# CNR-STIIMA-IRAS/rosdyn

Hardware: AMD Instinct MI355X
Metric: RNEA+regressor evals/s (6-DOF, batch 1e6) (higher is better)
Workload: dtype f64; 1 GPU; configs[1]: 6-DOF chain (ur10_like base_link->wrist_3_link, n=6, P=60), batch 1000000 samples per GPU, fp64 getJointTorque + dense getRegressor, inputs sample-major, Y layout stacked; samples_per_gpu=1000000, n_active=6, n_params=60, parallelism=sample-sharded x1

## Files before the change

### rosdyn_amd/csrc/rdyn_cholqr.hip

```cpp
#include <hip/hip_runtime.h>
#include <cstdint>
#include <type_traits>
#include "rdyn_device.h"
#include "rdyn_devmath.h"
#include "rdyn_kernels.h"
#include "rdyn_gram_common.h"
#include "rdyn_duo_common.h"
#include "rdyn_launch_util.h"

#ifndef RDYN_CHOLQR_AHEAD
#define RDYN_CHOLQR_AHEAD 2
#endif
#define DUO_BARRIER_LDS() asm volatile("s_waitcnt lgkmcnt(0)\n\ts_barrier" ::: "memory")
#define DUO_BARRIER() asm volatile("s_barrier" ::: "memory")

namespace
{

typedef const __attribute__((address_space(1))) double* GlobalD;

template <int NJ, bool ALLREV, int NPAIR, bool WGLOBAL, int XB, int KIN = 0>
__global__ __launch_bounds__(128 * NPAIR) void k_regressor_pgram(const RdynLdsGramArgs fa, const double* __restrict__ Wg, const int* __restrict__ run_flag)
{
  constexpr bool DIRECT = true;
  constexpr int NB = (10 * NJ + 1 + 15) / 16 + XB, NT = NB * (NB + 1) / 2, P = 10 * NJ;
  constexpr int SH = XB > 0 ? 0 : 16 * NB - (P + 1);
  constexpr int WB = WGLOBAL ? 0 : NT * 2048;
  if (run_flag && *run_flag == 0) return;
  extern __shared__ __attribute__((aligned(32))) char lds_raw[];
  const int lane = threadIdx.x & 63;
  const int wave = __builtin_amdgcn_readfirstlane(threadIdx.x >> 6);
  const bool sweeper = wave < NPAIR;
  const int pair = NPAIR == 4 ? (wave & 3) : NPAIR == 2 ? (wave & 1) : (wave < 3 ? wave : (wave == 3 ? 2 : wave - 4));
  if constexpr (!WGLOBAL)
  {
    double* const wl = (double*)lds_raw;
    for (int i = threadIdx.x; i < NT * 256; i += 128 * NPAIR) wl[i] = Wg[i];
    __syncthreads();
  }
  char* const tile = lds_raw + WB + (size_t)pair * fa.tile_bytes;
  const int n = fa.n_active;
  const int64_t t_mul = fa.tile_stride > 1 ? fa.tile_stride : 1;
  const int64_t n_tiles = ((fa.n_samples + 15) / 16 + t_mul - 1) / t_mul;
  const int64_t t_step = (int64_t)gridDim.x * NPAIR;
  const int64_t t_first = (int64_t)blockIdx.x * NPAIR + pair;
  const int64_t trips_raw = (n_tiles - (int64_t)blockIdx.x * NPAIR + t_step - 1) / t_step;
  const int64_t trips = trips_raw > 0 ? trips_raw : 0;

#ifndef RDYN_PGRAM_X_IDLE
#define RDYN_PGRAM_X_IDLE(wave_) true
#endif
#ifdef RDYN_PGRAM_X_NOSWEEP
  if (sweeper && RDYN_PGRAM_X_IDLE(wave))
  {
    if (KIN) DUO_BARRIER();
    for (int64_t it = 0; it < trips; ++it)
      for (int f = 0; f <= NJ; ++f) DUO_BARRIER_LDS();
  }
  else
#endif
  if (sweeper && KIN)
  {
    constexpr int XV = NJ <= 6 ? 21 : 12;
    constexpr int KIN_SLOTS = 3;
    const int KIN_SW = wave;
    char* const kin_tiles = lds_raw + WB;
    double* const kin_xch_base = (double*)(lds_raw + WB + (size_t)4 * fa.tile_bytes);
#include "rdyn_kin_sweepers.inc"
  }
  else if (sweeper)
  {
    ChainPtr c = as_const(fa.chain);
    const int s_loc = lane >> 2, k = lane & 3;
    const int r0 = k, r1 = k + 4;
    RDYN_DUO_INPUT_OFFSETS(fa, k, in_oa, in_ob);
    const int fB = 4;
    double nqa = 0.0, ndqa = 0.0, nddqa = 0.0, nqb = 0.0, ndqb = 0.0, nddqb = 0.0, nb0 = 0.0, nb1 = 0.0;
    auto fetch = [&](int64_t tile_index) {
      int64_t sx = tile_index * t_mul * 16 + s_loc;
      if (sx >= fa.n_samples) sx = fa.n_samples - 1;
      const int64_t o = sx * fa.in_ss;
      if (fa.bcol)
      {
        if (r0 < n) nb0 = fa.bcol[o + in_oa];
        if (r1 < n) nb1 = fa.bcol[o + in_ob];
      }
      if (k < n)
      {
        nqa = fa.q[o + in_oa];
        ndqa = fa.dq[o + in_oa];
        nddqa = fa.ddq[o + in_oa];
      }
      if (k + 4 < n)
      {
        nqb = fa.q[o + in_ob];
        ndqb = fa.dq[o + in_ob];
        nddqb = fa.ddq[o + in_ob];
      }
    };
    if (t_first < n_tiles) fetch(t_first);
    for (int64_t it = 0; it < trips; ++it)
    {
      const int64_t tl = t_first + it * t_step;
      const bool valid = tl < n_tiles && tl * t_mul * 16 + s_loc < fa.n_samples;
      const int m0idx = valid ? r0 : -2, m1idx = valid ? r1 : -2;
      const double qa = nqa, dqa = ndqa, ddqa = nddqa, qb = nqb, dqb = ndqb, ddqb = nddqb;
      const double tb0 = valid ? nb0 : 0.0, tb1 = valid ? nb1 : 0.0;
      if (tl + t_step < n_tiles) fetch(tl + t_step);
      double sna, csa, snb, csb;
      rdyn_sincos(qa, &sna, &csa);
      rdyn_sincos(qb, &snb, &csb);
      const double oca = 1.0 - csa, ocb = 1.0 - csb;
      V3 w = mk(0, 0, 0), vl = mk(0, 0, 0), al = mk(0, 0, 0);
      V3 lin = mk(-c->g[0], -c->g[1], -c->g[2]);
      V3 L0 = mk(0, 0, 0), A0 = mk(0, 0, 0), L1 = mk(0, 0, 0), A1 = mk(0, 0, 0);
#pragma unroll
      for (int f = 0; f < NJ; ++f)
      {
#include "rdyn_duo_link_body.inc"
      }
      if constexpr (XB > 0)
      {
#include "rdyn_duo_comp_cols.inc"
      }
      {
        char* const lb = tile + fa.lds_off_b + s_loc * 8;
        if (r0 < n) *(double*)(lb + r0 * 128) = tb0;
        if (r1 < n) *(double*)(lb + r1 * 128) = tb1;
      }
      DUO_BARRIER_LDS();
    }
  }
  else
  {
#ifdef RDYN_CHOLQR_MFMA_PRIO
    __builtin_amdgcn_s_setprio(RDYN_CHOLQR_MFMA_PRIO);
#endif
    const int cl = lane & 15, g = lane >> 4;
    constexpr int X0 = (P + SH) / 4, NX = 4 * NB - X0;
    const int K = XB > 0 ? fa.n_comp_cols : 0;
    int xoff[NX], xrow[NX];
#pragma unroll
    for (int i = 0; i < NX; ++i)
    {
      const int col = 4 * (X0 + i) + g - SH;
      int off = 0, row = -2;
      if (col >= P && col < P + K)
      {
        row = fa.comp_col_row[col - P];
        off = fa.lds_off_c + (col - P) * fa.comp_stride - row * 128;
      }
      else if (col == P + K)
      {
        off = fa.lds_off_b;
        row = -1;
      }
      xoff[i] = off + cl * 8;
      xrow[i] = row;
    }
    auto a_operand = [&](int cb1, int kk, int j) -> double {
      const int id = 4 * cb1 + kk, col = 4 * id + g - SH;
      double a = 0.0;
      if (id < X0 || (4 * id - SH < P && col < P))
      {
        if (col < 0) return 0.0;
        const int f = (col * 205) >> 11;
        constexpr int PAD = KIN ? KIN : 4;
        const int off = f * (640 * f + 640 + 80 * PAD) + (col - 10 * f) * (128 * f + 128 + 8 * PAD);
        if (j <= f) a = *(const double*)(tile + off + cl * 8 + j * 128);
      }
      else
      {
        const int i = id - X0;
        if (xrow[i] == -1 || xrow[i] == j) a = *(const double*)(tile + xoff[i] + j * 128);
      }
      return a;
    };
    d4 acc[NT];
#pragma unroll
    for (int t = 0; t < NT; ++t) acc[t] = (d4){0.0, 0.0, 0.0, 0.0};
    const char* const wl = lds_raw + lane * 8;
    GlobalD wgp = (GlobalD)Wg;
#ifdef RDYN_PGRAM_X_NOW
    auto wglob = [&](int blk_kk) -> double { return (double)(blk_kk + lane); };
#else
    auto wglob = [&](int blk_kk) -> double { return (wgp + blk_kk * 64)[lane]; };
#endif
    d4 D[NB];
    auto stage1 = [&](int j, int band) {
#pragma unroll
      for (int cb = 0; cb < NB; ++cb) D[cb] = (d4){0.0, 0.0, 0.0, 0.0};
      constexpr int AH = RDYN_CHOLQR_AHEAD;
      double ring[AH + 1][NB], aring[AH + 1];
      if constexpr (WGLOBAL) asm volatile("" : "+s"(wgp));
      auto load_row = [&](int r, double (&dst)[NB], double& adst) {
        const int c1 = band + (r >> 2), k4 = r & 3;
        adst = c1 < NB ? a_operand(c1, k4, j) : 0.0;
#pragma unroll
        for (int cb2 = 0; cb2 < NB; ++cb2)
        {
          dst[cb2] = 0.0;
          if (c1 < NB && cb2 >= c1)
          {
            if constexpr (WGLOBAL) dst[cb2] = wglob((cb2 * (cb2 + 1) / 2 + c1) * 4 + k4);
            else dst[cb2] = *(const double*)(wl + ((cb2 * (cb2 + 1) / 2 + c1) * 4 + k4) * 512);
          }
        }
      };
#pragma unroll
      for (int r = 0; r < AH; ++r) load_row(r, ring[r], aring[r]);
#pragma unroll
      for (int cb1 = 0; cb1 < NB; ++cb1)
      {
        if (cb1 < band) continue;
#pragma unroll
        for (int kk = 0; kk < 4; ++kk)
        {
          const int r = (cb1 - band) * 4 + kk;
          load_row(r + AH, ring[(r + AH) % (AH + 1)], aring[(r + AH) % (AH + 1)]);
          asm volatile("" ::: "memory");
          const double a = aring[r % (AH + 1)];
#pragma unroll
          for (int cb2 = cb1; cb2 < NB; ++cb2) D[cb2] = __builtin_amdgcn_mfma_f64_16x16x4f64(a, ring[r % (AH + 1)][cb2], D[cb2], 0, 0, 0);
        }
      }
    };
    auto stage2 = [&](int band) {
#pragma unroll
      for (int t = 0; t < 4; ++t)
      {
        int ti = 0;
#pragma unroll
        for (int cb = 0; cb < NB; ++cb)
#pragma unroll
          for (int rb = 0; rb <= cb; ++rb)
          {
            if (rb >= band) acc[ti] = __builtin_amdgcn_mfma_f64_16x16x4f64(D[rb][t], D[cb][t], acc[ti], 0, 0, 0);
            ++ti;
          }
      }
    };
    if (KIN) DUO_BARRIER();
    for (int64_t it = 0; it <= trips; ++it)
    {
#ifdef RDYN_PGRAM_X_NOMFMA
      const bool have = it > trips + 1;
#else
      const bool have = it > 0;
#endif
#pragma unroll
      for (int f = 0; f < NJ; ++f)
      {
        if (have) stage1(f, (SH + 10 * f) >> 4);
        if (it < trips) DUO_BARRIER_LDS();
        else asm volatile("s_waitcnt lgkmcnt(0)" ::: "memory");
        if (have) stage2((SH + 10 * f) >> 4);
      }
      if (it < trips) DUO_BARRIER_LDS();
    }
    DUO_BARRIER_LDS();
    double* red = (double*)lds_raw;
    for (int w = 0; w < NPAIR; ++w)
    {
      if (pair == w)
      {
#pragma unroll
        for (int t = 0; t < NT; ++t)
#pragma unroll
          for (int r = 0; r < 4; ++r)
          {
            const int idx = t * 256 + ((g + 4 * r) * 16 + cl);
            red[idx] = (w == 0) ? acc[t][r] : red[idx] + acc[t][r];
          }
      }
      asm volatile("s_waitcnt lgkmcnt(0)" ::: "memory");
      __builtin_amdgcn_s_barrier();
    }
  }
  if (sweeper)
    for (int w = 0; w < NPAIR + 1; ++w) __builtin_amdgcn_s_barrier();
  asm volatile("" ::: "memory");
  {
    const double* red = (const double*)lds_raw;
    double* slab = fa.slabs + (int64_t)blockIdx.x * (NT * 256);
    for (int i = threadIdx.x; i < NT * 256; i += 128 * NPAIR) slab[i] = red[i];
  }
}

template <int NB>
__global__ __launch_bounds__(256) void k_pgram_rows(const double* __restrict__ A, const double* __restrict__ bvec, int64_t rows, int64_t lda, int n_cols,
                                                    const double* __restrict__ Wg, double* __restrict__ slabs, const int* __restrict__ run_flag)
{
  constexpr int NT = NB * (NB + 1) / 2;
  if (run_flag && *run_flag == 0) return;
  extern __shared__ __attribute__((aligned(32))) char lds_raw[];
  const int lane = threadIdx.x & 63;
  const int wave = __builtin_amdgcn_readfirstlane(threadIdx.x >> 6);
  const int cl = lane & 15, g = lane >> 4;
  {
    double* const wl = (double*)lds_raw;
    for (int i = threadIdx.x; i < NT * 256; i += 256) wl[i] = Wg[i];
    __syncthreads();
  }
  d4 acc[NT];
#pragma unroll
  for (int t = 0; t < NT; ++t) acc[t] = (d4){0.0, 0.0, 0.0, 0.0};
  const char* const wl = lds_raw + lane * 8;
  const int64_t gstride = (int64_t)gridDim.x * 4 * 16;
  int64_t r0 = ((int64_t)blockIdx.x * 4 + wave) * 16;
  double cur[4 * NB], nxt[4 * NB];
  const double* const base = A + (int64_t)g * lda;
  const int id_b = bvec ? n_cols >> 2 : -1, g_b = n_cols & 3;
  auto load = [&](int64_t rbase, double (&v)[4 * NB]) {
    const int64_t r = rbase + cl;
    const bool in = r < rows;
    const double* pcol = base + r;
#pragma unroll
    for (int id = 0; id < 4 * NB; ++id)
    {
      double x = 0.0;
      if (in && 4 * id + g < n_cols) x = *pcol;
      if (id == id_b && in && g == g_b) x = bvec[r];
      v[id] = x;
      pcol += 4 * lda;
      asm volatile("" : "+v"(pcol));
    }
  };
  if (r0 < rows) load(r0, cur);
  while (r0 < rows)
  {
    const int64_t rn = r0 + gstride;
    constexpr bool LATE = NB >= 7;
    if (!LATE && rn < rows) load(rn, nxt);
    d4 D[NB];
#pragma unroll
    for (int cb = 0; cb < NB; ++cb) D[cb] = (d4){0.0, 0.0, 0.0, 0.0};
    {
      constexpr int AH = LATE ? 1 : 2;
      double ring[AH + 1][NB];
      auto load_row = [&](int r, double (&dst)[NB]) {
        const int c1 = r >> 2, k4 = r & 3;
#pragma unroll
        for (int cb2 = 0; cb2 < NB; ++cb2)
        {
          dst[cb2] = 0.0;
          if (c1 < NB && cb2 >= c1) dst[cb2] = *(const double*)(wl + ((cb2 * (cb2 + 1) / 2 + c1) * 4 + k4) * 512);
        }
      };
#pragma unroll
      for (int r = 0; r < AH; ++r) load_row(r, ring[r]);
#pragma unroll
      for (int cb1 = 0; cb1 < NB; ++cb1)
#pragma unroll
        for (int kk = 0; kk < 4; ++kk)
        {
          const int r = cb1 * 4 + kk;
          load_row(r + AH, ring[(r + AH) % (AH + 1)]);
          asm volatile("" ::: "memory");
          const double a = cur[r];
#pragma unroll
          for (int cb2 = cb1; cb2 < NB; ++cb2) D[cb2] = __builtin_amdgcn_mfma_f64_16x16x4f64(a, ring[r % (AH + 1)][cb2], D[cb2], 0, 0, 0);
        }
    }
    if (LATE)
    {
      asm volatile("" ::: "memory");
      if (rn < rows) load(rn, nxt);
// ... 1049 lines not shown
```

### rosdyn_amd/csrc/rdyn_duo_gram.hip

```cpp
#include <hip/hip_runtime.h>
#include <cstdint>
#include "rdyn_device.h"
#include "rdyn_devmath.h"
#include "rdyn_kernels.h"
#include "rdyn_gram_common.h"
#include "rdyn_duo_common.h"
#include "rdyn_launch_util.h"

#ifndef RDYN_DUO_SWEEP_UNROLL
#define RDYN_DUO_SWEEP_UNROLL 1
#endif

namespace
{

#ifdef RDYN_DUO_STAMPS
#ifndef RDYN_DUO_STAMP_TRIP
#define RDYN_DUO_STAMP_TRIP 7
#endif
#define DUO_STAMP_DECL unsigned long long st_wait = 0, st_t0 = __builtin_amdgcn_s_memtime(), st_tmp; long long st_it = -1; int st_n = 0
#define DUO_STAMP_TRIP(it_) st_it = (it_)
#define DUO_STAMP_MARK(t_) do { if (blockIdx.x == 0 && st_it == RDYN_DUO_STAMP_TRIP && (threadIdx.x & 63) == 0 && st_n < 32) fa.slabs[(int64_t)600 * 4096 + (threadIdx.x >> 6) * 32 + st_n++] = (double)((t_) - st_t0); } while (0)
#define DUO_STAMP_HERE(wait_lds) do { if (wait_lds) asm volatile("s_waitcnt lgkmcnt(0)" ::: "memory"); DUO_STAMP_MARK(__builtin_amdgcn_s_memtime()); } while (0)
#define DUO_BARRIER_LDS() do { st_tmp = __builtin_amdgcn_s_memtime(); DUO_STAMP_MARK(st_tmp); asm volatile("s_waitcnt lgkmcnt(0)\n\ts_barrier" ::: "memory"); const unsigned long long st_e = __builtin_amdgcn_s_memtime(); st_wait += st_e - st_tmp; DUO_STAMP_MARK(st_e); } while (0)
#define DUO_BARRIER() do { st_tmp = __builtin_amdgcn_s_memtime(); DUO_STAMP_MARK(st_tmp); asm volatile("s_barrier" ::: "memory"); const unsigned long long st_e = __builtin_amdgcn_s_memtime(); st_wait += st_e - st_tmp; DUO_STAMP_MARK(st_e); } while (0)
#define DUO_STAMP_OUT(NT_) do { if (lane == 0) { double* o = fa.slabs + ((int64_t)(256 + blockIdx.x) * (NT_ * 256)) + wave * 2; o[0] = (double)(__builtin_amdgcn_s_memtime() - st_t0); o[1] = (double)st_wait; } } while (0)
#else
#define DUO_STAMP_DECL
#define DUO_STAMP_TRIP(it_)
#define DUO_STAMP_HERE(wait_lds)
#define DUO_BARRIER_LDS() asm volatile("s_waitcnt lgkmcnt(0)\n\ts_barrier" ::: "memory")
#define DUO_BARRIER() asm volatile("s_barrier" ::: "memory")
#define DUO_STAMP_OUT(NT_)
#endif

typedef double d4h __attribute__((ext_vector_type(4), aligned(16)));

template <int NJ, bool DIRECT, int XB, bool ALLREV, int KIN = 0>
__global__ __launch_bounds__(KIN ? 768 : 512) void k_regressor_gram_duo(const RdynLdsGramArgs fa)
{
  constexpr int NB = (10 * NJ + 1 + 15) / 16 + XB;
  constexpr int NT = NB * (NB + 1) / 2;
  constexpr int P = 10 * NJ;
  extern __shared__ __attribute__((aligned(32))) char lds_raw[];
  const int lane = threadIdx.x & 63;
  const int wave = __builtin_amdgcn_readfirstlane(threadIdx.x >> 6);
  constexpr int NSW = KIN ? 8 : 4;
  const int pair = KIN ? (wave - NSW) & 3 : wave & 3;
  const bool sweeper = wave < NSW;
  char* const tile = lds_raw + (size_t)pair * fa.tile_bytes;
  const int n = fa.n_active;
  const int64_t t_mul = fa.tile_stride > 1 ? fa.tile_stride : 1;
  const int64_t n_tiles = ((fa.n_samples + 15) / 16 + t_mul - 1) / t_mul;
  const int64_t t_step = (int64_t)gridDim.x * 4;
  const int64_t t_first = (int64_t)blockIdx.x * 4 + pair;
  const int64_t trips_raw = (n_tiles - (int64_t)blockIdx.x * 4 + t_step - 1) / t_step;
  const int64_t trips = trips_raw > 0 ? trips_raw : 0;
  DUO_STAMP_DECL;

  if (sweeper && KIN)
  {
    constexpr int XV = NJ <= 6 ? (XB > 0 ? 30 : 21) : 12;
    constexpr int KIN_SLOTS = 2;
    const int KIN_SW = wave;
    char* const kin_tiles = lds_raw;
    double* const kin_xch_base = (double*)(lds_raw + (size_t)4 * fa.tile_bytes);
#include "rdyn_kin_sweepers.inc"
  }
  else if (sweeper)
  {
    ChainPtr c = as_const(fa.chain);
#ifdef RDYN_DUO_SWEEP_PRIO
    __builtin_amdgcn_s_setprio(RDYN_DUO_SWEEP_PRIO);
#endif
    const int s_loc = lane >> 2, k = lane & 3;
    const int r0 = k, r1 = k + 4;
    RDYN_DUO_INPUT_OFFSETS(fa, k, in_oa, in_ob);
    int fB = DIRECT ? 4 : NJ;
    if (!DIRECT)
      for (int f = NJ - 1; f >= 0; --f)
        if (fa.lds_m[f] >= 5) fB = f;
    double nqa = 0.0, ndqa = 0.0, nddqa = 0.0, nqb = 0.0, ndqb = 0.0, nddqb = 0.0, nb0 = 0.0, nb1 = 0.0;
    auto fetch = [&](int64_t tile_index) {
      int64_t sx = tile_index * t_mul * 16 + s_loc;
      if (sx >= fa.n_samples) sx = fa.n_samples - 1;
      const int64_t o = sx * fa.in_ss;
      if (fa.bcol)
      {
        if (r0 < n) nb0 = fa.bcol[o + in_oa];
        if (r1 < n) nb1 = fa.bcol[o + in_ob];
      }
      if (k < n)
      {
        nqa = fa.q[o + in_oa];
        ndqa = fa.dq[o + in_oa];
        nddqa = fa.ddq[o + in_oa];
      }
      if (k + 4 < n)
      {
        nqb = fa.q[o + in_ob];
        ndqb = fa.dq[o + in_ob];
        nddqb = fa.ddq[o + in_ob];
      }
    };
    if (t_first < n_tiles) fetch(t_first);
    for (int64_t it = 0; it < trips; ++it)
    {
      const int64_t tl = t_first + it * t_step;
      const bool valid = tl < n_tiles && tl * t_mul * 16 + s_loc < fa.n_samples;
      const int m0idx = valid ? r0 : -2, m1idx = valid ? r1 : -2;
      const double qa = nqa, dqa = ndqa, ddqa = nddqa, qb = nqb, dqb = ndqb, ddqb = nddqb;
      const double tb0 = valid ? nb0 : 0.0, tb1 = valid ? nb1 : 0.0;
      if (tl + t_step < n_tiles) fetch(tl + t_step);
      double sna, csa, snb, csb;
      rdyn_sincos(qa, &sna, &csa);
      rdyn_sincos(qb, &snb, &csb);
      const double oca = 1.0 - csa, ocb = 1.0 - csb;

      V3 w = mk(0, 0, 0), vl = mk(0, 0, 0), al = mk(0, 0, 0);
      V3 lin = mk(-c->g[0], -c->g[1], -c->g[2]);
      V3 L0 = mk(0, 0, 0), A0 = mk(0, 0, 0), L1 = mk(0, 0, 0), A1 = mk(0, 0, 0);
      if constexpr (DIRECT)
      {
#pragma unroll
        for (int f = 0; f < NJ; ++f)
        {
#include "rdyn_duo_link_body.inc"
        }
      }
      else
      {
#pragma unroll 1
        for (int f = 0; f < NJ; ++f)
        {
#include "rdyn_duo_link_body.inc"
        }
      }
      if (XB > 0 || fa.n_comps > 0)
      {
#include "rdyn_duo_comp_cols.inc"
      }
      {
        char* const lb = tile + fa.lds_off_b + s_loc * 8;
        if (r0 < n) *(double*)(lb + r0 * 128) = tb0;
        if (r1 < n) *(double*)(lb + r1 * 128) = tb1;
      }
      DUO_BARRIER_LDS();
    }
  }
  else
  {
#ifdef RDYN_DUO_MFMA_PRIO
    __builtin_amdgcn_s_setprio(RDYN_DUO_MFMA_PRIO);
#endif
    const int cl = lane & 15, g = lane >> 4;
    int colbase[NB], colm[NB], collo[NB];
    const int K = XB > 0 ? fa.n_comp_cols : 0;
    const int KF = K;
#pragma unroll
    for (int cb = 0; cb < NB; ++cb)
    {
      const int pp = 16 * cb + cl;
      const int pl = pp - KF - 1;
      const int p = pp < KF ? P + pp : (pp == KF ? P + K : (pl >= P ? P + K + 1 : 10 * (NJ - 1 - pl / 10) + pl % 10));
      int base = 0, hi = 0, lo = 0;
      if (p < P)
      {
        const int f = p / 10;
        base = fa.lds_off[f] + (p - 10 * f) * fa.lds_stride[f];
        hi = fa.lds_m[f];
      }
      else if (p < P + K)
      {
        lo = fa.comp_col_row[p - P];
        hi = lo + 1;
        base = fa.lds_off_c + (p - P) * fa.comp_stride - lo * 128;
      }
      else if (p == P + K)
      {
        base = fa.lds_off_b;
        hi = n;
      }
      colbase[cb] = base + g * 32;
      colm[cb] = hi;
      collo[cb] = lo;
    }
    d4 acc[NT];
#pragma unroll
    for (int t = 0; t < NT; ++t) acc[t] = (d4){0.0, 0.0, 0.0, 0.0};
    auto lds_group = [&](int j, int band, d4* op) {
#pragma unroll
      for (int cb = 0; cb < NB; ++cb)
      {
        d4 x = (d4){0.0, 0.0, 0.0, 0.0};
        if (cb <= band && j < colm[cb] && j >= collo[cb]) x = *(const d4h*)(tile + colbase[cb] + j * 128);
        op[cb] = x;
      }
    };
    auto mfma_band = [&](const d4* op, int band) {
#pragma unroll
      for (int t = 0; t < 4; ++t)
      {
        int ti = 0;
#pragma unroll
        for (int cb = 0; cb < NB; ++cb)
#pragma unroll
          for (int rb = 0; rb <= cb; ++rb)
          {
#ifdef RDYN_DUO_4X4_TIMING
            if (cb <= band)
            {
              acc[ti][0] = __builtin_amdgcn_mfma_f64_4x4x4f64(op[rb][t], op[cb][t], acc[ti][0], 0, 0, 0);
              acc[ti][1] = __builtin_amdgcn_mfma_f64_4x4x4f64(op[rb][t], op[cb][t], acc[ti][1], 0, 0, 0);
              acc[ti][2] = __builtin_amdgcn_mfma_f64_4x4x4f64(op[rb][t], op[cb][t], acc[ti][2], 0, 0, 0);
              if (rb != cb) acc[ti][3] = __builtin_amdgcn_mfma_f64_4x4x4f64(op[rb][t], op[cb][t], acc[ti][3], 0, 0, 0);
            }
#else
            if (cb <= band) acc[ti] = __builtin_amdgcn_mfma_f64_16x16x4f64(op[rb][t], op[cb][t], acc[ti], 0, 0, 0);
#endif
            ++ti;
          }
      }
    };
    constexpr bool ONEBUF = (NJ >= 7 && XB > 0) || KIN != 0;
    d4 opa[NB], opb[ONEBUF ? 1 : NB];
    if (KIN) DUO_BARRIER();
    for (int64_t it = 0; it <= trips; ++it)
    {
      DUO_STAMP_TRIP(it);
      const bool have = it > 0;
      if (have) lds_group(0, (KF + 10 * NJ) >> 4, opa);
#pragma unroll
      for (int f = 0; f < NJ; ++f)
      {
        d4* const cur = (ONEBUF || !(f & 1)) ? opa : opb;
        d4* const nxt = (ONEBUF || (f & 1)) ? opa : opb;
        if (it < trips) DUO_BARRIER_LDS();
        else asm volatile("s_waitcnt lgkmcnt(0)" ::: "memory");
        if (have)
        {
          if constexpr (ONEBUF)
          {
            mfma_band(cur, (KF + 10 * (NJ - f)) >> 4);
            if (f + 1 < NJ) lds_group(f + 1, (KF + 10 * (NJ - f - 1)) >> 4, nxt);
          }
          else
          {
            if (f + 1 < NJ) lds_group(f + 1, (KF + 10 * (NJ - f - 1)) >> 4, nxt);
            mfma_band(cur, (KF + 10 * (NJ - f)) >> 4);
          }
        }
      }
      if (it < trips) DUO_BARRIER_LDS();
    }

    DUO_STAMP_OUT(NT);
    DUO_BARRIER_LDS();
    double* red = (double*)lds_raw;
    const int cw = wave - NSW;
    for (int w = 0; w < 4; ++w)
    {
      if (cw == w)
      {
#pragma unroll
        for (int t = 0; t < NT; ++t)
#pragma unroll
          for (int r = 0; r < 4; ++r)
          {
            const int idx = t * 256 + ((g + 4 * r) * 16 + cl);
            red[idx] = (w == 0) ? acc[t][r] : red[idx] + acc[t][r];
          }
      }
      asm volatile("s_waitcnt lgkmcnt(0)" ::: "memory");
      __builtin_amdgcn_s_barrier();
    }
  }
  if (sweeper)
  {
    DUO_STAMP_OUT(NT);
    for (int w = 0; w < 5; ++w) __builtin_amdgcn_s_barrier();
  }
  asm volatile("" ::: "memory");
  {
    const double* red = (const double*)lds_raw;
    double* slab = fa.slabs + (int64_t)blockIdx.x * (NT * 256);
    for (int i = threadIdx.x; i < NT * 256; i += (KIN ? 768 : 512)) slab[i] = red[i];
  }
}

template <int NJ, bool DIRECT, int XB, bool ALLREV = false, int KIN = 0>
hipError_t launch_duo_nj2(const RdynLdsGramArgs& a, int blocks, size_t lds_bytes, hipStream_t st)
{
  hipError_t e = opt_in_lds_once<k_regressor_gram_duo<NJ, DIRECT, XB, ALLREV, KIN>>();
  if (e != hipSuccess) return e;
  hipLaunchKernelGGL((k_regressor_gram_duo<NJ, DIRECT, XB, ALLREV, KIN>), dim3(blocks), dim3(KIN ? 768 : 512), lds_bytes, st, a);
  return hipGetLastError();
}
template <int NJ>
hipError_t launch_duo_nj(const RdynLdsGramArgs& a, int blocks, size_t lds_bytes, hipStream_t st)
{
  bool direct = a.n_active == NJ;
  for (int f = 0; direct && f < NJ; ++f) direct = a.lds_m[f] == f + 1 && a.first_col[f] == 10 * f && a.lds_stride[f] == (16 * (f + 1) + 4) * 8;
  const int xb = a.n_comp_cols > 0 ? 1 : 0;
  if (a.sweep_lanes)
  {
    bool compact = a.n_active == NJ;
    for (int f = 0; compact && f < NJ; ++f) compact = a.lds_m[f] == f + 1 && a.first_col[f] == 10 * f && a.lds_stride[f] == (16 * (f + 1) + 2) * 8;
    if constexpr (NJ <= 6)
    {
      if (direct && xb == 0) return a.all_revolute ? launch_duo_nj2<NJ, true, 0, true, 4>(a, blocks, lds_bytes, st) : launch_duo_nj2<NJ, true, 0, false, 4>(a, blocks, lds_bytes, st);
      if constexpr (NJ >= 5)
        if (direct && xb == 1) return a.all_revolute ? launch_duo_nj2<NJ, true, 1, true, 4>(a, blocks, lds_bytes, st) : launch_duo_nj2<NJ, true, 1, false, 4>(a, blocks, lds_bytes, st);
    }
    else if (compact && xb == 0)
      return a.all_revolute ? launch_duo_nj2<NJ, true, 0, true, 2>(a, blocks, lds_bytes, st) : launch_duo_nj2<NJ, true, 0, false, 2>(a, blocks, lds_bytes, st);
    return hipErrorInvalidValue;
  }
  if (xb == 0 && direct && a.all_revolute) return launch_duo_nj2<NJ, true, 0, true>(a, blocks, lds_bytes, st);
  if (xb == 0) return direct ? launch_duo_nj2<NJ, true, 0>(a, blocks, lds_bytes, st) : launch_duo_nj2<NJ, false, 0>(a, blocks, lds_bytes, st);
  if constexpr (NJ >= 5)
  {
    if (xb == 1 && direct && a.all_revolute) return launch_duo_nj2<NJ, true, 1, true>(a, blocks, lds_bytes, st);
    if (xb == 1) return direct ? launch_duo_nj2<NJ, true, 1>(a, blocks, lds_bytes, st) : launch_duo_nj2<NJ, false, 1>(a, blocks, lds_bytes, st);
  }
  return hipErrorInvalidValue;
}
}

bool rdyn_regressor_gram_duo_supported(int n_cols) { return n_cols >= 20 && n_cols <= 70; }
int rdyn_regressor_gram_duo_kin_pad(int n_joints, int n_comp_cols)
{
  if (n_joints >= 2 && n_joints <= 6) return (n_comp_cols == 0 || n_joints >= 5) ? 4 : 0;
  return (n_joints == 7 && n_comp_cols == 0) ? 2 : 0;
}
bool rdyn_regressor_gram_duo_supports_components(int n_cols, int n_comp_cols)
{
  if (!rdyn_regressor_gram_duo_supported(n_cols) || n_comp_cols < 0 || n_comp_cols > 96) return false;
  if (n_comp_cols == 0) return true;
  const int nb1 = (n_cols + 1 + 15) / 16 + 1;
  return n_cols >= 50 && n_cols + n_comp_cols + 1 <= 16 * nb1;
}

hipError_t rdyn_launch_regressor_gram_duo(int n_cols, const RdynLdsGramArgs& a, int blocks, size_t lds_bytes, hipStream_t st)
{
#define CALL(N) launch_duo_nj<N>(a, blocks, lds_bytes, st)
  RDYN_DISPATCH_JOINTS_2_7(n_cols / 10, CALL)
#undef CALL
}
```

### rosdyn_amd/csrc/rdyn_kin_link_body.inc

```
        asm volatile("" : "+s"(c));
        JointRef J = c->j[g];
        const int type = J.type;
        const bool rev = ALLREV || type == RDYN_REVOLUTE, pri = !ALLREV && type == RDYN_PRISMATIC;
        const double qf = q_[g], dqf = dq_[g], ddqf = ddq_[g];
        {
          const int64_t oj = o_next + (int64_t)fa.in_map[g] * fa.in_sj;
          q_[g] = fa.q[oj];
          dq_[g] = fa.dq[oj];
          ddq_[g] = fa.ddq[oj];
        }
        const double sn = rev ? sn_[g] : 0.0, oc = rev ? oc_[g] : 0.0;
        const double qp = pri ? qf : 0.0;
        double R[9];
#pragma unroll
        for (int i = 0; i < 9; ++i) R[i] = fma(sn, J.B[i], fma(oc, J.C[i], J.A[i]));
        const V3 tt = ALLREV ? ld3(J.t) : axpy(ld3(J.t), ld3(J.up), qp);
        {
          const V3 wn = rotT(R, w);
          const V3 vn = rotT(R, vl + cross(w, tt));
          const V3 aln = rotT(R, al);
          const V3 an = rotT(R, lin + cross(al, tt));
          w = wn; vl = vn; al = aln; lin = an;
        }
        const V3 u = ld3(J.u);
        {
          const double dqr = rev ? dqf : 0.0, ddqr = rev ? ddqf : 0.0, dqp = pri ? dqf : 0.0, ddqp = pri ? ddqf : 0.0;
          const V3 wxu = cross(w, u);
          if constexpr (ALLREV)
            lin = axpy(lin, cross(vl, u), dqr);
          else
            lin = axpy(axpy(axpy(lin, cross(vl, u), dqr), wxu, dqp), u, ddqp);
          al = axpy(axpy(al, wxu, dqr), u, ddqr);
          w = axpy(w, u, dqr);
          if constexpr (!ALLREV) vl = axpy(vl, u, dqp);
        }
        const V3 d = lin + cross(w, vl);
        double* const o = xch + (g & 1) * (XV * 64);
        if constexpr (XV == 12)
        {
          o[0] = sn; o[64] = oc; o[128] = qp;
          o[192] = w.x; o[256] = w.y; o[320] = w.z;
          o[384] = al.x; o[448] = al.y; o[512] = al.z;
          o[576] = d.x; o[640] = d.y; o[704] = d.z;
        }
        else
        {
          const double wxy = w.x * w.y, wxz = w.x * w.z, wyz = w.y * w.z;
          const double wxx = w.x * w.x, wyy = w.y * w.y, wzz = w.z * w.z;
#pragma unroll
          for (int i = 0; i < 9; ++i) o[i * 64] = R[i];
          o[576] = tt.x; o[640] = tt.y; o[704] = tt.z;
          o[768] = w.x; o[832] = w.y; o[896] = w.z;
          o[960] = al.x; o[1024] = al.y; o[1088] = al.z;
          o[1152] = d.x; o[1216] = d.y; o[1280] = d.z;
          if constexpr (XV == 30)
          {
            o[1344] = -(wyy + wzz); o[1408] = wxy - al.z; o[1472] = wxz + al.y;
            o[1536] = wxy + al.z; o[1600] = -(wxx + wzz); o[1664] = wyz - al.x;
            o[1728] = wxz - al.y; o[1792] = wyz + al.x; o[1856] = -(wxx + wyy);
          }
        }
```

### rosdyn_amd/csrc/rdyn_kin_sweepers.inc

```
#ifndef DUO_STAMP_TRIP
#define DUO_STAMP_TRIP(it_)
#endif
#ifndef DUO_STAMP_HERE
#define DUO_STAMP_HERE(wait_lds)
#endif
    ChainPtr c = as_const(fa.chain);
    const int sub = lane >> 4, s_loc = lane & 15;
    char* const tile = kin_tiles + (size_t)sub * fa.tile_bytes;
    double* const xch = kin_xch_base + lane;
    const int64_t t_mine = (int64_t)blockIdx.x * 4 + sub;
    auto sample_offset = [&](int64_t tile_index) -> int64_t {
      if (tile_index >= n_tiles) tile_index = n_tiles - 1;
      int64_t sx = tile_index * t_mul * 16 + s_loc;
      if (sx >= fa.n_samples) sx = fa.n_samples - 1;
      return sx * fa.in_ss;
    };
    if (KIN_SW == 0)
    {
      double q_[NJ], dq_[NJ], ddq_[NJ];
      {
        const int64_t o = sample_offset(t_mine);
#pragma unroll
        for (int j = 0; j < NJ; ++j)
        {
          const int64_t oj = o + (int64_t)fa.in_map[j] * fa.in_sj;
          q_[j] = fa.q[oj];
          dq_[j] = fa.dq[oj];
          ddq_[j] = fa.ddq[oj];
        }
      }
      V3 w = mk(0, 0, 0), vl = mk(0, 0, 0), al = mk(0, 0, 0), lin = mk(-c->g[0], -c->g[1], -c->g[2]);
      int64_t o_next = sample_offset(t_mine + t_step);
      double sn_[NJ], oc_[NJ];
#define RDYN_KIN_ONE_SINCOS(j_)                                                                     \
  do                                                                                               \
  {                                                                                                \
    double sn1_, cs1_;                                                                             \
    rdyn_sincos_small(q_[j_], &sn1_, &cs1_);                                                       \
    if (__builtin_expect(!(fabs(q_[j_]) <= 1048576.0), 0))                                         \
    {                                                                                              \
      const DuoSinCos big_ = duo_sincos_cold(q_[j_]);                                              \
      sn1_ = big_.sn;                                                                              \
      cs1_ = big_.cs;                                                                              \
    }                                                                                              \
    sn_[j_] = sn1_;                                                                                \
    oc_[j_] = 1.0 - cs1_;                                                                          \
  } while (0)
#pragma unroll
      for (int j = 0; j < NJ; ++j) RDYN_KIN_ONE_SINCOS(j);
      {
        constexpr int g = 0;
#include "rdyn_kin_link_body.inc"
      }
      DUO_BARRIER_LDS();
      for (int64_t it = 0; it < trips; ++it)
      {
        DUO_STAMP_TRIP(it);
#pragma unroll
        for (int f = 0; f < NJ; ++f)
        {
          if (f + 1 < NJ)
          {
            const int g = f + 1;
#include "rdyn_kin_link_body.inc"
          }
          else
          {
#pragma unroll
            for (int j = 0; j < NJ; ++j) RDYN_KIN_ONE_SINCOS(j);
          }
          DUO_BARRIER_LDS();
        }
        w = mk(0, 0, 0); vl = mk(0, 0, 0); al = mk(0, 0, 0); lin = mk(-c->g[0], -c->g[1], -c->g[2]);
        o_next = sample_offset(t_mine + (it + 2) * t_step);
        {
          constexpr int g = 0;
#include "rdyn_kin_link_body.inc"
        }
        DUO_BARRIER_LDS();
      }
    }
    else
    {
      constexpr int S = KIN_SLOTS;
      int r[S];
      int64_t ob[S];
#pragma unroll
      for (int k = 0; k < S; ++k)
      {
        r[k] = fa.sw_rows[3 * (KIN_SW - 1) + k];
        ob[k] = r[k] < 8 ? (int64_t)fa.in_map[r[k]] * fa.in_sj : 0;
      }
      double nb[S], nq[S], nd[S];
#pragma unroll
      for (int k = 0; k < S; ++k) nb[k] = nq[k] = nd[k] = 0.0;
      auto fetch = [&](int64_t tile_index) {
        const int64_t o = sample_offset(tile_index);
#pragma unroll
        for (int k = 0; k < S; ++k)
        {
          if (fa.bcol && r[k] < 8) nb[k] = fa.bcol[o + ob[k]];
          if ((XB > 0 || fa.n_comps > 0) && r[k] < 8)
          {
            nq[k] = fa.q[o + ob[k]];
            nd[k] = fa.dq[o + ob[k]];
          }
        }
      };
      fetch(t_mine);
      DUO_BARRIER();
      for (int64_t it = 0; it < trips; ++it)
      {
        DUO_STAMP_TRIP(it);
        const int64_t tl = t_mine + it * t_step;
        const bool valid = tl < n_tiles && tl * t_mul * 16 + s_loc < fa.n_samples;
        double tb[S], qr[S], dqr[S];
#pragma unroll
        for (int k = 0; k < S; ++k)
        {
          tb[k] = valid ? nb[k] : 0.0;
          qr[k] = nq[k];
          dqr[k] = nd[k];
        }
        fetch(tl + t_step);
        V3 L[S], A[S];
#pragma unroll
        for (int k = 0; k < S; ++k) L[k] = A[k] = mk(0, 0, 0);
        int col_off = 0;
#pragma unroll 1
        for (int f = 0; f < NJ; ++f)
        {
          const double* const xi = xch + (f & 1) * (XV * 64);
          double R[9], b00, b01, b02, b10, b11, b12, b20, b21, b22;
          V3 tt, w, al, d;
          if constexpr (XV == 12)
          {
            asm volatile("" : "+s"(c));
            JointRef J = c->j[f];
            const double sn = xi[0], oc = xi[64], qp = xi[128];
            w = mk(xi[192], xi[256], xi[320]);
            al = mk(xi[384], xi[448], xi[512]);
            d = mk(xi[576], xi[640], xi[704]);
#pragma unroll
            for (int i = 0; i < 9; ++i) R[i] = fma(sn, J.B[i], fma(oc, J.C[i], J.A[i]));
            tt = ALLREV ? ld3(J.t) : axpy(ld3(J.t), ld3(J.up), qp);
            const double wxy = w.x * w.y, wxz = w.x * w.z, wyz = w.y * w.z;
            const double wxx = w.x * w.x, wyy = w.y * w.y, wzz = w.z * w.z;
            b00 = -(wyy + wzz); b01 = wxy - al.z; b02 = wxz + al.y;
            b10 = wxy + al.z; b11 = -(wxx + wzz); b12 = wyz - al.x;
            b20 = wxz - al.y; b21 = wyz + al.x; b22 = -(wxx + wyy);
          }
          else
          {
#pragma unroll
            for (int i = 0; i < 9; ++i) R[i] = xi[i * 64];
            tt = mk(xi[576], xi[640], xi[704]);
            w = mk(xi[768], xi[832], xi[896]);
            al = mk(xi[960], xi[1024], xi[1088]);
            d = mk(xi[1152], xi[1216], xi[1280]);
            if constexpr (XV == 30)
            {
              b00 = xi[1344]; b01 = xi[1408]; b02 = xi[1472];
              b10 = xi[1536]; b11 = xi[1600]; b12 = xi[1664];
              b20 = xi[1728]; b21 = xi[1792]; b22 = xi[1856];
            }
            else
            {
              const double wxy = w.x * w.y, wxz = w.x * w.z, wyz = w.y * w.z;
              const double wxx = w.x * w.x, wyy = w.y * w.y, wzz = w.z * w.z;
              b00 = -(wyy + wzz); b01 = wxy - al.z; b02 = wxz + al.y;
              b10 = wxy + al.z; b11 = -(wxx + wzz); b12 = wyz - al.x;
              b20 = wxz - al.y; b21 = wyz + al.x; b22 = -(wxx + wyy);
            }
          }
#pragma unroll
          for (int k = 0; k < S; ++k)
            if (f > r[k])
            {
              const V3 nL = rotT(R, L[k] + cross(A[k], tt));
              A[k] = rotT(R, A[k]);
              L[k] = nL;
            }
          bool starts = false;
#pragma unroll
          for (int k = 0; k < S; ++k) starts = starts || f == r[k];
          if (starts)
          {
            asm volatile("" : "+s"(c));
            JointRef J = c->j[f];
            const int type = J.type;
            const bool rev = ALLREV || type == RDYN_REVOLUTE, pri = !ALLREV && type == RDYN_PRISMATIC;
            const V3 u = ld3(J.u);
            const V3 sl = mk((pri && valid) ? u.x : 0.0, (pri && valid) ? u.y : 0.0, (pri && valid) ? u.z : 0.0);
            const V3 sa = mk((rev && valid) ? u.x : 0.0, (rev && valid) ? u.y : 0.0, (rev && valid) ? u.z : 0.0);
#pragma unroll
            for (int k = 0; k < S; ++k)
              if (f == r[k])
              {
                L[k] = sl;
                A[k] = sa;
              }
          }
          double y[S][10];
#pragma unroll
          for (int k = 0; k < S; ++k)
            if (f >= r[k])
            {
              const V3 Lk = L[k], Ak = A[k];
              const V3 dxA = cross(d, Ak), x = cross(Ak, w);
              y[k][0] = dot(Lk, d);
              y[k][1] = fma(Lk.x, b00, fma(Lk.y, b10, fma(Lk.z, b20, dxA.x)));
              y[k][2] = fma(Lk.x, b01, fma(Lk.y, b11, fma(Lk.z, b21, dxA.y)));
              y[k][3] = fma(Lk.x, b02, fma(Lk.y, b12, fma(Lk.z, b22, dxA.z)));
              y[k][4] = fma(Ak.x, al.x, x.x * w.x);
              y[k][5] = fma(Ak.x, al.y, fma(Ak.y, al.x, fma(x.x, w.y, x.y * w.x)));
              y[k][6] = fma(Ak.x, al.z, fma(Ak.z, al.x, fma(x.x, w.z, x.z * w.x)));
              y[k][7] = fma(Ak.y, al.y, x.y * w.y);
              y[k][8] = fma(Ak.y, al.z, fma(Ak.z, al.y, fma(x.y, w.z, x.z * w.y)));
              y[k][9] = fma(Ak.z, al.z, x.z * w.z);
            }
          DUO_BARRIER_LDS();
          const int stride = (16 * (f + 1) + KIN) * 8;
          char* const lf = tile + col_off + s_loc * 8;
          col_off += 10 * stride;
#pragma unroll
          for (int k = 0; k < S; ++k)
            if (f >= r[k])
            {
#pragma unroll
              for (int p = 0; p < 10; ++p) *(double*)(lf + p * stride + r[k] * 128) = y[k][p];
            }
          DUO_STAMP_HERE(0);
          DUO_STAMP_HERE(1);
        }
        if (XB > 0 || fa.n_comps > 0)
        {
          int col = 0;
          for (int ci = 0; ci < fa.n_comps; ++ci)
          {
            const int type = fa.comps[ci].type, jc = fa.comps[ci].joint;
            const int cols = type == RDYN_COMP_FRICTION2 ? 3 : 2;
            bool mine = false;
            double qv = 0.0, dv = 0.0;
#pragma unroll
            for (int k = 0; k < S; ++k)
              if (jc == r[k])
              {
                mine = true;
                qv = qr[k];
                dv = dqr[k];
              }
            if (mine)
            {
              double row[3] = {0.0, 0.0, 0.0};
              if (type == RDYN_COMP_SPRING)
              {
                row[0] = qv;
                row[1] = 1.0;
              }
              else
              {
                const double vmax = fa.comps[ci].max_velocity, vmin = fa.comps[ci].min_velocity;
                const double omega = fmin(fmax(dv, -vmax), vmax);
                double sg;
                if (type == RDYN_COMP_FRICTION1)
                  sg = fmin(fmax(omega / vmin, -1.0), 1.0);
                else
                  sg = (omega == 0.0) ? 0.0 : (omega > vmin ? 1.0 : (omega < -vmin ? -1.0 : omega / vmin));
                row[0] = sg;
                row[1] = omega;
                row[2] = omega * omega * sg;
              }
              char* const lc = tile + fa.lds_off_c + col * fa.comp_stride + jc * fa.comp_row_step + s_loc * 8;
              for (int e = 0; e < cols; ++e) *(double*)(lc + e * fa.comp_stride) = valid ? row[e] : 0.0;
            }
            col += cols;
          }
        }
        {
          char* const lb = tile + fa.lds_off_b + s_loc * 8;
#pragma unroll
          for (int k = 0; k < S; ++k)
            if (r[k] < 8) *(double*)(lb + r[k] * 128) = tb[k];
        }
        DUO_BARRIER_LDS();
      }
    }
```

Measured before the change: 2.182 billion evals/s.

## Split Gram MFMA tile consumption across two consumer wave groups

Adds a CSPLIT mode for the KIN sweeper path of the duo Gram kernel. The triangular MFMA tiles are partitioned between two groups of four consumer waves by a compile-time load-balanced ownership mask, so each wave issues about half the MFMAs and only loads the operand columns it needs. The block grows to 1024 threads and the sweepers drop to one kinematic slot, with dq/ddq refills shifted across the previous and next sample so register live ranges shrink. In exchange the kernel has more waves per block and uses more registers and LDS, which may lower occupancy, and the reduction loop now runs over both halves.

```diff
diff --git a/rosdyn_amd/csrc/rdyn_cholqr.hip b/rosdyn_amd/csrc/rdyn_cholqr.hip
--- a/rosdyn_amd/csrc/rdyn_cholqr.hip
+++ b/rosdyn_amd/csrc/rdyn_cholqr.hip
@@ -63,6 +63,7 @@
   {
     constexpr int XV = NJ <= 6 ? 21 : 12;
     constexpr int KIN_SLOTS = 3;
+    constexpr int KIN_REFILL_SHIFT = 0;
     const int KIN_SW = wave;
     char* const kin_tiles = lds_raw + WB;
     double* const kin_xch_base = (double*)(lds_raw + WB + (size_t)4 * fa.tile_bytes);
diff --git a/rosdyn_amd/csrc/rdyn_duo_gram.hip b/rosdyn_amd/csrc/rdyn_duo_gram.hip
--- a/rosdyn_amd/csrc/rdyn_duo_gram.hip
+++ b/rosdyn_amd/csrc/rdyn_duo_gram.hip
@@ -1,5 +1,6 @@
 #include <hip/hip_runtime.h>
 #include <cstdint>
+#include <type_traits>
 #include "rdyn_device.h"
 #include "rdyn_devmath.h"
 #include "rdyn_kernels.h"
@@ -7,6 +8,9 @@
 #include "rdyn_duo_common.h"
 #include "rdyn_launch_util.h"
 
+#ifndef RDYN_DUO_CSPLIT
+#define RDYN_DUO_CSPLIT 2
+#endif
 #ifndef RDYN_DUO_SWEEP_UNROLL
 #define RDYN_DUO_SWEEP_UNROLL 1
 #endif
@@ -34,11 +38,43 @@
 #define DUO_STAMP_OUT(NT_)
 #endif
 
+struct DuoSplit
+{
+  unsigned own[2];
+  int need_from[2][8];
+  int load[2];
+};
+constexpr DuoSplit duo_split(int NJ, int XB)
+{
+  const int NB = (10 * NJ + 1 + 15) / 16 + XB, KF = XB > 0 ? 2 * NJ : 0;
+  DuoSplit s = {{0u, 0u}, {{99, 99, 99, 99, 99, 99, 99, 99}, {99, 99, 99, 99, 99, 99, 99, 99}}, {0, 0}};
+  int tiles[2] = {0, 0}, ti = 0;
+  for (int cb = 0; cb < NB; ++cb)
+  {
+    int weight = 0;
+    for (int f = 0; f < NJ; ++f) weight += ((KF + 10 * (NJ - f)) >> 4) >= cb;
+    for (int rb = 0; rb <= cb; ++rb, ++ti)
+    {
+      const int h = s.load[0] != s.load[1] ? s.load[1] < s.load[0] : tiles[1] < tiles[0];
+      s.own[h] |= 1u << ti;
+      s.load[h] += weight;
+      ++tiles[h];
+      if (s.need_from[h][rb] > cb) s.need_from[h][rb] = cb;
+      if (s.need_from[h][cb] > cb) s.need_from[h][cb] = cb;
+    }
+  }
+  return s;
+}
+static_assert(duo_split(6, 0).load[0] == 16 && duo_split(6, 0).load[1] == 17, "6 joints: 64 / 68 MFMAs per tile");
+static_assert((duo_split(7, 0).own[0] ^ duo_split(7, 0).own[1]) == (1u << 15) - 1, "every tile has exactly one owner");
+
 typedef double d4h __attribute__((ext_vector_type(4), aligned(16)));
 
-template <int NJ, bool DIRECT, int XB, bool ALLREV, int KIN = 0>
-__global__ __launch_bounds__(KIN ? 768 : 512) void k_regressor_gram_duo(const RdynLdsGramArgs fa)
-{
+template <int NJ, bool DIRECT, int XB, bool ALLREV, int KIN = 0, int CSPLIT = 1>
+__global__ __launch_bounds__(KIN ? 512 + 256 * CSPLIT : 512) void k_regressor_gram_duo(const RdynLdsGramArgs fa)
+{
+  static_assert(CSPLIT == 1 || (CSPLIT == 2 && KIN != 0), "the consumer split belongs to the one-lane-per-sample sweepers");
+  constexpr int NTHREADS = KIN ? 512 + 256 * CSPLIT : 512;
   constexpr int NB = (10 * NJ + 1 + 15) / 16 + XB;
   constexpr int NT = NB * (NB + 1) / 2;
   constexpr int P = 10 * NJ;
@@ -61,7 +97,8 @@
   if (sweeper && KIN)
   {
     constexpr int XV = NJ <= 6 ? (XB > 0 ? 30 : 21) : 12;
-    constexpr int KIN_SLOTS = 2;
+    constexpr int KIN_SLOTS = CSPLIT == 2 ? 1 : 2;
+    constexpr int KIN_REFILL_SHIFT = CSPLIT == 2 ? NJ / 2 : 0;
     const int KIN_SW = wave;
     char* const kin_tiles = lds_raw;
     double* const kin_xch_base = (double*)(lds_raw + (size_t)4 * fa.tile_bytes);
@@ -185,6 +222,10 @@
       colm[cb] = hi;
       collo[cb] = lo;
     }
+    auto consume = [&](auto half_c) {
+    constexpr int HALF = decltype(half_c)::value;
+    constexpr DuoSplit SPLIT = duo_split(NJ, XB);
+    constexpr unsigned OWN = CSPLIT == 1 ? ~0u : SPLIT.own[HALF];
     d4 acc[NT];
 #pragma unroll
     for (int t = 0; t < NT; ++t) acc[t] = (d4){0.0, 0.0, 0.0, 0.0};
@@ -193,7 +234,7 @@
       for (int cb = 0; cb < NB; ++cb)
       {
         d4 x = (d4){0.0, 0.0, 0.0, 0.0};
-        if (cb <= band && j < colm[cb] && j >= collo[cb]) x = *(const d4h*)(tile + colbase[cb] + j * 128);
+        if (cb <= band && (CSPLIT == 1 || band >= SPLIT.need_from[HALF][cb]) && j < colm[cb] && j >= collo[cb]) x = *(const d4h*)(tile + colbase[cb] + j * 128);
         op[cb] = x;
       }
     };
@@ -216,7 +257,7 @@
               if (rb != cb) acc[ti][3] = __builtin_amdgcn_mfma_f64_4x4x4f64(op[rb][t], op[cb][t], acc[ti][3], 0, 0, 0);
             }
 #else
-            if (cb <= band) acc[ti] = __builtin_amdgcn_mfma_f64_16x16x4f64(op[rb][t], op[cb][t], acc[ti], 0, 0, 0);
+            if (cb <= band && ((OWN >> ti) & 1u)) acc[ti] = __builtin_amdgcn_mfma_f64_16x16x4f64(op[rb][t], op[cb][t], acc[ti], 0, 0, 0);
 #endif
             ++ti;
           }
@@ -257,23 +298,29 @@
     DUO_STAMP_OUT(NT);
     DUO_BARRIER_LDS();
     double* red = (double*)lds_raw;
-    const int cw = wave - NSW;
+    const int cw = (wave - NSW) & 3;
     for (int w = 0; w < 4; ++w)
     {
       if (cw == w)
       {
 #pragma unroll
         for (int t = 0; t < NT; ++t)
-#pragma unroll
-          for (int r = 0; r < 4; ++r)
+          if ((OWN >> t) & 1u)
           {
-            const int idx = t * 256 + ((g + 4 * r) * 16 + cl);
-            red[idx] = (w == 0) ? acc[t][r] : red[idx] + acc[t][r];
+#pragma unroll
+            for (int r = 0; r < 4; ++r)
+            {
+              const int idx = t * 256 + ((g + 4 * r) * 16 + cl);
+              red[idx] = (w == 0) ? acc[t][r] : red[idx] + acc[t][r];
+            }
           }
       }
       asm volatile("s_waitcnt lgkmcnt(0)" ::: "memory");
       __builtin_amdgcn_s_barrier();
     }
+    };
+    if (CSPLIT == 1 || wave - NSW < 4) consume(std::integral_constant<int, 0>{});
+    else consume(std::integral_constant<int, 1>{});
   }
   if (sweeper)
   {
@@ -284,16 +331,25 @@
   {
     const double* red = (const double*)lds_raw;
     double* slab = fa.slabs + (int64_t)blockIdx.x * (NT * 256);
-    for (int i = threadIdx.x; i < NT * 256; i += (KIN ? 768 : 512)) slab[i] = red[i];
-  }
+    for (int i = threadIdx.x; i < NT * 256; i += NTHREADS) slab[i] = red[i];
+  }
+}
+
+constexpr int duo_csplit(int NJ, int XB, bool ALLREV, int KIN)
+{
+  if (KIN == 0 || RDYN_DUO_CSPLIT != 2 || !ALLREV) return 1;
+  return (XB > 0 && NJ <= 5) ? 1 : 2;
 }
 
 template <int NJ, bool DIRECT, int XB, bool ALLREV = false, int KIN = 0>
 hipError_t launch_duo_nj2(const RdynLdsGramArgs& a, int blocks, size_t lds_bytes, hipStream_t st)
 {
-  hipError_t e = opt_in_lds_once<k_regressor_gram_duo<NJ, DIRECT, XB, ALLREV, KIN>>();
+  constexpr int CSPLIT = duo_csplit(NJ, XB, ALLREV, KIN);
+  for (int w = 0; CSPLIT == 2 && w < 7; ++w)
+    if (a.sw_rows[3 * w + 1] != 99) return hipErrorInvalidValue;
+  hipError_t e = opt_in_lds_once<k_regressor_gram_duo<NJ, DIRECT, XB, ALLREV, KIN, CSPLIT>>();
   if (e != hipSuccess) return e;
-  hipLaunchKernelGGL((k_regressor_gram_duo<NJ, DIRECT, XB, ALLREV, KIN>), dim3(blocks), dim3(KIN ? 768 : 512), lds_bytes, st, a);
+  hipLaunchKernelGGL((k_regressor_gram_duo<NJ, DIRECT, XB, ALLREV, KIN, CSPLIT>), dim3(blocks), dim3(KIN ? 512 + 256 * CSPLIT : 512), lds_bytes, st, a);
   return hipGetLastError();
 }
 template <int NJ>
diff --git a/rosdyn_amd/csrc/rdyn_kin_link_body.inc b/rosdyn_amd/csrc/rdyn_kin_link_body.inc
--- a/rosdyn_amd/csrc/rdyn_kin_link_body.inc
+++ b/rosdyn_amd/csrc/rdyn_kin_link_body.inc
@@ -6,8 +6,18 @@
         {
           const int64_t oj = o_next + (int64_t)fa.in_map[g] * fa.in_sj;
           q_[g] = fa.q[oj];
-          dq_[g] = fa.dq[oj];
-          ddq_[g] = fa.ddq[oj];
+          if constexpr (KIN_REFILL_SHIFT == 0)
+          {
+            dq_[g] = fa.dq[oj];
+            ddq_[g] = fa.ddq[oj];
+          }
+          else
+          {
+            const int jr = (g + NJ - KIN_REFILL_SHIFT) % NJ;
+            const int64_t or_ = (g >= KIN_REFILL_SHIFT ? o_next : o_cur) + (int64_t)fa.in_map[jr] * fa.in_sj;
+            dq_[jr] = fa.dq[or_];
+            ddq_[jr] = fa.ddq[or_];
+          }
         }
         const double sn = rev ? sn_[g] : 0.0, oc = rev ? oc_[g] : 0.0;
         const double qp = pri ? qf : 0.0;
diff --git a/rosdyn_amd/csrc/rdyn_kin_sweepers.inc b/rosdyn_amd/csrc/rdyn_kin_sweepers.inc
--- a/rosdyn_amd/csrc/rdyn_kin_sweepers.inc
+++ b/rosdyn_amd/csrc/rdyn_kin_sweepers.inc
@@ -31,6 +31,7 @@
       }
       V3 w = mk(0, 0, 0), vl = mk(0, 0, 0), al = mk(0, 0, 0), lin = mk(-c->g[0], -c->g[1], -c->g[2]);
       int64_t o_next = sample_offset(t_mine + t_step);
+      int64_t o_cur = sample_offset(t_mine);
       double sn_[NJ], oc_[NJ];
 #define RDYN_KIN_ONE_SINCOS(j_)                                                                     \
   do                                                                                               \
@@ -72,6 +73,7 @@
           DUO_BARRIER_LDS();
         }
         w = mk(0, 0, 0); vl = mk(0, 0, 0); al = mk(0, 0, 0); lin = mk(-c->g[0], -c->g[1], -c->g[2]);
+        o_cur = o_next;
         o_next = sample_offset(t_mine + (it + 2) * t_step);
         {
           constexpr int g = 0;
```

Result: slower. 1.877 billion evals/s (-14.0%).
